# Arash-san/YinYang-Game-AlphaZero

Hardware: AMD Instinct MI355X
Metric: self-play positions/sec (+ MCTS node-expansions/sec) at 800 sims, 8x8 board (higher is better)
Workload: dtype f16x3; 1 GPU; 8x8 board, 800 sims/move, 4096 concurrent games per GPU, frozen random-init 128x10 net (seed 0), copied boards, reference_quirks=False, staggered start plies; tree_arithmetic=f32 PUCT + u64 bitboards, nn_dtype=f16x3, evaluation_reuse=False, parallelism=episode-sharded x1, lanes_per_gpu=2, hipgraph=True

## Files before the change

include/yy_engine.h:

```cpp
#ifndef YY_ENGINE_H
#define YY_ENGINE_H

#include <stdint.h>

#ifdef __cplusplus
extern "C" {
#endif

#define YY_OK 0
#define YY_E_INVALID (-1)
#define YY_E_UNSUPPORTED (-2)
#define YY_E_NOMEM (-3)
#define YY_E_HIP (-4)
#define YY_E_STATE (-5)
#define YY_E_ARENA (-6)

#define YY_FLAG_ROWCOL 1u
#define YY_FLAG_ALIASED 2u
#define YY_FLAG_REUSE_PASS_VALUE 4u

#define YY_FLAG_REUSE_TRANSPOSITIONS 8u
#define YY_FLAG_KEEP_EVALUATIONS 16u

#define YY_FLAG_EVAL_SYMMETRY 32u

#define YY_FLAG_FORCED_PLAYOUTS 64u

#define YY_FLAG_FPU_REDUCTION 128u

typedef void *yy_stream_t;

const char *yy_last_error(void);
int yy_version(void);


int yy_rules_valid_mask(const int8_t *boards, const int8_t *players, int G, int R, int C,
                        uint32_t flags, uint8_t *out_mask, yy_stream_t stream);

int yy_rules_step(int8_t *boards, int8_t *players, const int32_t *actions, int G, int R, int C,
                  uint32_t flags, uint8_t *placed, yy_stream_t stream);

int yy_rules_game_ended(const int8_t *boards, const int8_t *players, int G, int R, int C,
                        uint32_t flags, double *out, int32_t *counts, yy_stream_t stream);

int yy_encode_planes(const int8_t *boards, int G, int R, int C, float *out, yy_stream_t stream);

int yy_encode_planes_sym(const int8_t *boards, int G, int R, int C, uint64_t seed, float *out, yy_stream_t stream);
int yy_eval_symmetry(const int8_t *boards, int G, int R, int C, uint64_t seed, int8_t *out, yy_stream_t stream);

int yy_rules_mask_terminal_bb(const uint64_t *black, const uint64_t *white, int G, int R, int C,
                              uint32_t flags, uint64_t *mask_p1, uint64_t *mask_m1,
                              int8_t *result, yy_stream_t stream);

int yy_pack_boards(const int8_t *boards, int G, int R, int C, uint64_t *black, uint64_t *white,
                   yy_stream_t stream);
int yy_unpack_boards(const uint64_t *black, const uint64_t *white, int G, int R, int C,
                     int8_t *boards, yy_stream_t stream);


typedef struct yy_mcts_config {
    int32_t G;
    int32_t R, C;
    int32_t max_sims;
    float cpuct;
    uint32_t flags;
    int64_t edges_per_game;
    int64_t nodes_per_game;
    int32_t leaves_per_step;
    uint64_t symmetry_seed;
    double forced_playouts;
    float fpu_reduction;
    float fpu_reduction_root;
} yy_mcts_config;


typedef struct yy_mcts yy_mcts;

int yy_mcts_create(const yy_mcts_config *cfg, yy_mcts **out);
int yy_mcts_destroy(yy_mcts *ctx);
int yy_mcts_memory_bytes(const yy_mcts *ctx, uint64_t *out);
int yy_mcts_set_num_sims(yy_mcts *ctx, int32_t num_sims);
int yy_mcts_set_sim_budgets(yy_mcts *ctx, const int32_t *budgets_dev);

int yy_mcts_advance(yy_mcts *ctx, const int32_t *actions, int32_t *kept_visits, yy_stream_t stream);

int yy_mcts_begin(yy_mcts *ctx, const int8_t *boards, const int8_t *root_players,
                  const uint8_t *active, float *planes_out, yy_stream_t stream);

int yy_mcts_expand_root(yy_mcts *ctx, const float *policy, const double *noise, double eps,
                        yy_stream_t stream);

int yy_mcts_select(yy_mcts *ctx, float *planes_out, uint8_t *needs_eval, yy_stream_t stream);

int yy_mcts_expand_backup(yy_mcts *ctx, const float *policy, const float *value,
                          yy_stream_t stream);

int yy_mcts_step(yy_mcts *ctx, const float *policy, const float *value, float *planes_out,
                 uint8_t *needs_eval, yy_stream_t stream);

int yy_mcts_root_counts(yy_mcts *ctx, int32_t *counts, float *child_w, float *child_p,
                        yy_stream_t stream);

int yy_mcts_root_policy(yy_mcts *ctx, int temperature_is_zero, double *pi, yy_stream_t stream);

int yy_mcts_root_stats(yy_mcts *ctx, int32_t *visits, double *value_sum, yy_stream_t stream);

int yy_mcts_get_boards(yy_mcts *ctx, int8_t *boards, yy_stream_t stream);

int yy_mcts_status(yy_mcts *ctx, int32_t *n_overflow, uint64_t *counters);
int yy_mcts_reset_counters(yy_mcts *ctx, yy_stream_t stream);
int yy_mcts_forced_descents(yy_mcts *ctx, uint64_t *out);
int yy_book_insert(const uint64_t *keys, int n, int R, int C, uint32_t *meta, uint64_t *table_keys, int64_t cap,
                   int32_t *slot_of, yy_stream_t stream);
int yy_mcts_set_book(yy_mcts *ctx, const uint32_t *meta, const uint64_t *keys, const float *value, const float *policy,
                     int64_t cap, int max_stones);
int yy_mcts_cache_clear(yy_mcts *ctx, yy_stream_t stream);
int yy_mcts_set_shared_evaluations(yy_mcts *ctx, uint32_t *meta, uint64_t *keys, float *value, float *policy, int64_t slots,
                                   uint32_t *stamp);
int yy_mcts_shared_evaluations_clear(yy_mcts *ctx, yy_stream_t stream);
int yy_mcts_shared_counters(yy_mcts *ctx, uint64_t *out);
int yy_mcts_set_shared_evaluations_replacing(yy_mcts *ctx, uint64_t *claim, uint32_t *last_hit, uint64_t *keys, float *value,
                                             float *policy, int64_t slots, uint32_t *stamp, uint64_t *sweep_state);
int yy_mcts_shared_evaluations_sweep(yy_mcts *ctx, int64_t high_water_slots, yy_stream_t stream);
int yy_mcts_shared_counters_ex(yy_mcts *ctx, uint64_t *out);

int yy_nn_bias_act_bf16(void *x, const float *bias, const void *residual, int64_t rows, int C,
                        int relu, yy_stream_t stream);

int yy_nn_tower_bf16(const float *planes, const void *weights, const float *bias, void *out, int G,
                     int R, int C, int channels, int n_layers, yy_stream_t stream);

int yy_nn_tower_heads_bf16(const float *planes, const void *weights, const float *bias,
                           void *out_heads, int G, int R, int C, int channels, int n_layers,
                           yy_stream_t stream);

int yy_nn_tower_f32(const float *planes, const void *weights, const float *bias, float *out, int G,
                    int R, int C, int channels, int n_layers, yy_stream_t stream);

int yy_nn_head_finish_bf16(const void *h, int G, int A, int H, const float *w2, const float *b2,
                           float *policy, float *value, yy_stream_t stream);

int yy_nn_tower_f16x3_regs(const float *planes, const void *weights, const void *head_w, const float *bias,
                           float *out, float *out_heads, const int32_t *rows, const int32_t *n_rows, int G,
                           int R, int C, int channels, int n_layers, int weight_exp, int head_exp,
                           int act_exp, yy_stream_t stream);

int yy_nn_tower_g(const float *planes, const void *weights, const void *head_w, const float *bias, const float *head_bias,
                  float *out, float *out_heads, const int32_t *rows, const int32_t *n_rows, int G, int R, int C,
                  int channels, int n_layers, int weight_exp, int head_exp, int act_exp, int nb, int boards, int gate_lo,
                  int gate_hi, int layout, yy_stream_t stream);
int yy_nn_tower_g_forms(int channels, int *nb_out);
int yy_nn_tower_g_relu_check(uint32_t start, uint32_t count, uint32_t *counts, yy_stream_t stream);

int yy_nn_fc_heads_f16x3(const float *feats, const void *wpk, const float *bias, const int32_t *jobs, int n_jobs,
                         float *logits, float *hidden, const int32_t *n_rows, int G, int K, int A, int H,
                         int weight_exp, int act_exp, yy_stream_t stream);

int yy_nn_head_finish_f32(const float *logits, const float *hidden, int G, int A, int H, const float *w2,
                          const float *b2, const int32_t *rows, const int32_t *n_rows, float *policy,
                          float *value, yy_stream_t stream);

int yy_compact_rows(const uint8_t *flags, int G, int32_t *rows, int32_t *n, yy_stream_t stream);

int yy_selfplay_root_noise(uint64_t seed, const int64_t *game_id, const int32_t *ply, const uint8_t *draw,
                           const uint8_t *mask, int G, int A, double alpha, double *noise, yy_stream_t stream);

int yy_selfplay_sample_actions(uint64_t seed, const int64_t *game_id, const int32_t *ply,
                               const uint8_t *searching, const double *pi, const uint8_t *mask, int G, int A,
                               int temperature_threshold, int32_t *action, yy_stream_t stream);

int yy_selfplay_draw_budgets(uint64_t seed, const int64_t *game_id, const int32_t *ply, const uint8_t *searching, int G,
                             double p_full, int full_sims, int fast_sims, int32_t *budgets, uint8_t *is_full,
                             yy_stream_t stream);

typedef struct yy_selfplay_config {
    uint64_t seed;
    double dirichlet_alpha;
    double dirichlet_epsilon;
    double full_search_probability;
    int32_t temperature_threshold;
    int32_t num_simulations;
    int32_t fast_simulations;
    int32_t reserved;
    int64_t example_capacity;
} yy_selfplay_config;

typedef struct yy_selfplay_run yy_selfplay_run;

int yy_selfplay_run_create(yy_mcts *ctx, const yy_selfplay_config *cfg, yy_selfplay_run **out);
int yy_selfplay_run_destroy(yy_selfplay_run *run);
int yy_selfplay_run_arm(yy_mcts *ctx, yy_selfplay_run *run, int64_t num_games, int64_t first_game_index, int64_t stride,
                        float *planes, uint8_t *needs_eval, yy_stream_t stream);
int yy_mcts_step_selfplay(yy_mcts *ctx, yy_selfplay_run *run, const float *policy, const float *value, float *planes,
                          uint8_t *needs_eval, yy_stream_t stream);
int yy_selfplay_run_counters(yy_selfplay_run *run, uint64_t *out, yy_stream_t stream);
int yy_selfplay_run_examples(yy_selfplay_run *run, int64_t first, int64_t count, int8_t *states, float *policies,
                             float *values, int64_t *game_id, int64_t *ply, yy_stream_t stream);

#ifdef __cplusplus
}
#endif
#endif
```

yinyang-game-alphazero_amd/_lib.py:

```python
import ctypes as C
import os
import subprocess

_HERE = os.path.dirname(os.path.abspath(__file__))
CSRC = os.path.join(_HERE, "csrc")
SO = os.path.join(CSRC, "libyy_hip.so")
HEADER = os.path.normpath(os.path.join(_HERE, "..", "include", "yy_engine.h"))

YY_OK = 0
YY_E_ARENA = -6
FLAG_ROWCOL = 1
FLAG_ALIASED = 2
FLAG_REUSE_PASS_VALUE = 4
FLAG_REUSE_TRANSPOSITIONS = 8
FLAG_KEEP_EVALUATIONS = 16
FLAG_EVAL_SYMMETRY = 32
FLAG_FORCED_PLAYOUTS = 64
FLAG_FPU_REDUCTION = 128

HIPCC_FLAGS = ["--offload-arch=gfx950", "-O3", "-std=c++17", "-fPIC", "-shared",
               "-ffp-contract=off", "-fno-fast-math", "-Wall", "-Wno-unused-function"]


class YYError(RuntimeError):
    def __init__(self, code, msg):
        super().__init__(f"libyy_hip: status {code}: {msg}")
        self.code = code


class MctsConfig(C.Structure):
    _fields_ = [("G", C.c_int32), ("R", C.c_int32), ("C", C.c_int32), ("max_sims", C.c_int32),
                ("cpuct", C.c_float), ("flags", C.c_uint32), ("edges_per_game", C.c_int64),
                ("nodes_per_game", C.c_int64), ("leaves_per_step", C.c_int32), ("symmetry_seed", C.c_uint64),
                ("forced_playouts", C.c_double), ("fpu_reduction", C.c_float), ("fpu_reduction_root", C.c_float)]


class SelfPlayConfig(C.Structure):
    _fields_ = [("seed", C.c_uint64), ("dirichlet_alpha", C.c_double), ("dirichlet_epsilon", C.c_double),
                ("full_search_probability", C.c_double), ("temperature_threshold", C.c_int32),
                ("num_simulations", C.c_int32), ("fast_simulations", C.c_int32), ("reserved", C.c_int32),
                ("example_capacity", C.c_int64)]


def build(force=False, verbose=False):
    srcs = [os.path.join(CSRC, f) for f in ("yy_engine.hip", "yy_nn_epilogue.hip", "yy_tower.hip", "yy_tower_f32.hip",
                                            "yy_tower_h3r.hip", "yy_tower_g.hip", "yy_fc_heads.hip", "yy_selfplay.hip",
                                            "yy_selfplay_move.hip", "yy_shared_table.hip", "yy_bitboard.h", "yy_common.h", "yy_tree.h",
                                            "yy_draws.h")] + [HEADER]
    if not force and os.path.exists(SO) and all(os.path.getmtime(SO) >= os.path.getmtime(s) for s in srcs):
        return SO
    hipcc = os.environ.get("HIPCC", "/opt/rocm/bin/hipcc")
    tmp = f"{SO}.{os.getpid()}.tmp"
    cmd = [hipcc] + HIPCC_FLAGS + ["-o", tmp] + [s for s in srcs if s.endswith(".hip")]
    if verbose:
        print(" ".join(cmd).replace(tmp, SO))
    try:
        subprocess.check_call(cmd)
        os.replace(tmp, SO)
    finally:
        if os.path.exists(tmp):
            os.remove(tmp)
    return SO


_LIB = None
_vp = C.c_void_p
_SIGS = {
    "yy_rules_valid_mask": [_vp, _vp, C.c_int, C.c_int, C.c_int, C.c_uint32, _vp, _vp],
    "yy_rules_step": [_vp, _vp, _vp, C.c_int, C.c_int, C.c_int, C.c_uint32, _vp, _vp],
    "yy_rules_game_ended": [_vp, _vp, C.c_int, C.c_int, C.c_int, C.c_uint32, _vp, _vp, _vp],
    "yy_encode_planes": [_vp, C.c_int, C.c_int, C.c_int, _vp, _vp],
    "yy_encode_planes_sym": [_vp, C.c_int, C.c_int, C.c_int, C.c_uint64, _vp, _vp],
    "yy_eval_symmetry": [_vp, C.c_int, C.c_int, C.c_int, C.c_uint64, _vp, _vp],
    "yy_rules_mask_terminal_bb": [_vp, _vp, C.c_int, C.c_int, C.c_int, C.c_uint32, _vp, _vp, _vp, _vp],
    "yy_pack_boards": [_vp, C.c_int, C.c_int, C.c_int, _vp, _vp, _vp],
    "yy_unpack_boards": [_vp, _vp, C.c_int, C.c_int, C.c_int, _vp, _vp],
    "yy_mcts_create": [C.POINTER(MctsConfig), C.POINTER(_vp)],
    "yy_mcts_destroy": [_vp],
    "yy_mcts_memory_bytes": [_vp, C.POINTER(C.c_uint64)],
    "yy_mcts_set_num_sims": [_vp, C.c_int32],
    "yy_mcts_set_sim_budgets": [_vp, _vp],
    "yy_mcts_advance": [_vp, _vp, _vp, _vp],
    "yy_mcts_begin": [_vp, _vp, _vp, _vp, _vp, _vp],
    "yy_mcts_expand_root": [_vp, _vp, _vp, C.c_double, _vp],
    "yy_mcts_select": [_vp, _vp, _vp, _vp],
    "yy_mcts_expand_backup": [_vp, _vp, _vp, _vp],
    "yy_mcts_step": [_vp, _vp, _vp, _vp, _vp, _vp],
    "yy_mcts_root_counts": [_vp, _vp, _vp, _vp, _vp],
    "yy_mcts_root_policy": [_vp, C.c_int, _vp, _vp],
    "yy_mcts_root_stats": [_vp, _vp, _vp, _vp],
    "yy_mcts_get_boards": [_vp, _vp, _vp],
    "yy_mcts_status": [_vp, C.POINTER(C.c_int32), C.POINTER(C.c_uint64)],
    "yy_mcts_reset_counters": [_vp, _vp],
    "yy_mcts_forced_descents": [_vp, C.POINTER(C.c_uint64)],
    "yy_mcts_cache_clear": [_vp, _vp],
    "yy_book_insert": [_vp, C.c_int, C.c_int, C.c_int, _vp, _vp, C.c_int64, _vp, _vp],
    "yy_mcts_set_book": [_vp, _vp, _vp, _vp, _vp, C.c_int64, C.c_int],
    "yy_mcts_set_shared_evaluations": [_vp, _vp, _vp, _vp, _vp, C.c_int64, _vp],
    "yy_mcts_shared_evaluations_clear": [_vp, _vp],
    "yy_mcts_shared_counters": [_vp, C.POINTER(C.c_uint64)],
    "yy_mcts_set_shared_evaluations_replacing": [_vp, _vp, _vp, _vp, _vp, _vp, C.c_int64, _vp, _vp],
    "yy_mcts_shared_evaluations_sweep": [_vp, C.c_int64, _vp],
    "yy_mcts_shared_counters_ex": [_vp, C.POINTER(C.c_uint64)],
    "yy_nn_bias_act_bf16": [_vp, _vp, _vp, C.c_int64, C.c_int, C.c_int, _vp],
    "yy_nn_tower_bf16": [_vp, _vp, _vp, _vp, C.c_int, C.c_int, C.c_int, C.c_int, C.c_int, _vp],
    "yy_nn_tower_heads_bf16": [_vp, _vp, _vp, _vp, C.c_int, C.c_int, C.c_int, C.c_int, C.c_int, _vp],
    "yy_nn_head_finish_bf16": [_vp, C.c_int, C.c_int, C.c_int, _vp, _vp, _vp, _vp, _vp],
    "yy_nn_tower_f32": [_vp, _vp, _vp, _vp, C.c_int, C.c_int, C.c_int, C.c_int, C.c_int, _vp],
    "yy_nn_head_finish_f32": [_vp, _vp, C.c_int, C.c_int, C.c_int, _vp, _vp, _vp, _vp, _vp, _vp, _vp],
    "yy_compact_rows": [_vp, C.c_int, _vp, _vp, _vp],
    "yy_nn_tower_f16x3_regs": [_vp, _vp, _vp, _vp, _vp, _vp, _vp, _vp, C.c_int, C.c_int, C.c_int, C.c_int, C.c_int, C.c_int, C.c_int,
                               C.c_int, _vp],
    "yy_nn_tower_g_forms": [C.c_int, C.POINTER(C.c_int)],
    "yy_nn_tower_g_relu_check": [C.c_uint32, C.c_uint32, _vp, _vp],
    "yy_nn_tower_g": [_vp, _vp, _vp, _vp, _vp, _vp, _vp, _vp, _vp, C.c_int, C.c_int, C.c_int, C.c_int, C.c_int, C.c_int, C.c_int,
                      C.c_int, C.c_int, C.c_int, C.c_int, C.c_int, C.c_int, _vp],
    "yy_nn_fc_heads_f16x3": [_vp, _vp, _vp, _vp, C.c_int, _vp, _vp, _vp, C.c_int, C.c_int, C.c_int, C.c_int, C.c_int, C.c_int, _vp],
    "yy_selfplay_root_noise": [C.c_uint64, _vp, _vp, _vp, _vp, C.c_int, C.c_int, C.c_double, _vp, _vp],
    "yy_selfplay_sample_actions": [C.c_uint64, _vp, _vp, _vp, _vp, _vp, C.c_int, C.c_int, C.c_int, _vp, _vp],
    "yy_selfplay_draw_budgets": [C.c_uint64, _vp, _vp, _vp, C.c_int, C.c_double, C.c_int, C.c_int, _vp, _vp, _vp],
    "yy_selfplay_run_create": [_vp, C.POINTER(SelfPlayConfig), C.POINTER(_vp)],
    "yy_selfplay_run_destroy": [_vp],
    "yy_selfplay_run_arm": [_vp, _vp, C.c_int64, C.c_int64, C.c_int64, _vp, _vp, _vp],
    "yy_mcts_step_selfplay": [_vp, _vp, _vp, _vp, _vp, _vp, _vp],
    "yy_selfplay_run_counters": [_vp, _vp, _vp],
    "yy_selfplay_run_examples": [_vp, C.c_int64, C.c_int64, _vp, _vp, _vp, _vp, _vp, _vp],
    "yy_version": [],
}


def exported_symbols():
    return sorted(list(_SIGS) + ["yy_last_error"])


def lib():
    global _LIB
    if _LIB is None:
        if not os.path.exists(SO):
            raise YYError(-100, f"{SO} is missing: run __graft_entry__.build() (hipcc --offload-arch=gfx950); "
                                "there is no CPU fallback for the product path")
        L = C.CDLL(SO)
        for name, args in _SIGS.items():
            fn = getattr(L, name)
            fn.argtypes = args
            fn.restype = C.c_int
        L.yy_last_error.restype = C.c_char_p
        L.yy_last_error.argtypes = []
        _LIB = L
    return _LIB


def check(status):
    if status != YY_OK:
        raise YYError(status, lib().yy_last_error().decode())
    return status
```

yinyang-game-alphazero_amd/csrc/yy_fc_heads.hip:

```cpp
#include <hip/hip_runtime.h>
#include <math.h>
#include <stdint.h>

#include "../../include/yy_engine.h"

typedef __attribute__((ext_vector_type(8))) _Float16 f16x8;
typedef __attribute__((ext_vector_type(2))) _Float16 f16x2;
typedef __attribute__((ext_vector_type(4))) float f32x4;
typedef __attribute__((ext_vector_type(2))) float f32x2;
typedef __attribute__((ext_vector_type(4))) unsigned int u32x4;
typedef __attribute__((ext_vector_type(2))) unsigned int u32x2;

#include "yy_common.h"

namespace fch {

constexpr int KC = 128, RS = 288;

__device__ __forceinline__ void split_pair(const f32x2 a, uint32_t &hi, uint32_t &lo) {
    const f16x2 h = __builtin_convertvector(a, f16x2);
    const f32x2 r = a - __builtin_convertvector(h, f32x2);
    const f16x2 l = __builtin_convertvector(r, f16x2);
    hi = __builtin_bit_cast(uint32_t, h);
    lo = __builtin_bit_cast(uint32_t, l);
}

struct Job {
    int head, out0, nout, wchunk;
};

template <int ROWS>
__global__ void __launch_bounds__(256, 2)
k_fc_heads(const float *__restrict__ feats, const unsigned char *__restrict__ wpk, const float *__restrict__ bias,
           const Job *__restrict__ jobs, int n_jobs, float *__restrict__ logits, float *__restrict__ hidden,
           const int *__restrict__ n_rows, int G, int K, int A, int H, float in_scale, float out_scale) {
    constexpr int PART_BYTES = ROWS * RS, STAGE_BYTES = 2 * PART_BYTES, NBR = ROWS / 16, NI = ROWS / 8;
    __shared__ __attribute__((aligned(256))) unsigned char lds[2 * STAGE_BYTES];
    const int n_live = n_rows ? min(*n_rows, G) : G;
    const int tile = blockIdx.x / n_jobs, jb = blockIdx.x - tile * n_jobs;
    const int r0 = tile * ROWS;
    if (r0 >= n_live) return;
    const Job job = jobs[jb];
    const int lane = threadIdx.x & 63, wave = __builtin_amdgcn_readfirstlane(threadIdx.x >> 6);
    const int n16 = lane & 15, kg = lane >> 4;
    const int n_chunks = (K + KC - 1) / KC;
    const bool active = wave * 16 < job.nout;

    const int sq = threadIdx.x & 31, sr = threadIdx.x >> 5;
    auto stage_load = [&](f32x4 (&fr)[NI], int c) {
        const int k = c * KC + sq * 4;
        const int kc = k < K ? k : 0;
        const float km = k < K ? 1.0f : 0.0f;
#pragma unroll
        for (int i = 0; i < NI; i++) {
            const int row = min(r0 + sr + 8 * i, n_live - 1);
            fr[i] = *(const f32x4 *)(feats + ((size_t)row * 2 + job.head) * K + kc) * km;
        }
    };
    auto stage_store = [&](const f32x4 (&fr)[NI], int s) {
        unsigned char *base = lds + s * STAGE_BYTES + sq * 8;
#pragma unroll
        for (int i = 0; i < NI; i++) {
            const f32x4 v = fr[i] * in_scale;
            uint32_t h01, l01, h23, l23;
            split_pair((f32x2){v[0], v[1]}, h01, l01);
            split_pair((f32x2){v[2], v[3]}, h23, l23);
            *(u32x2 *)(base + (sr + 8 * i) * RS) = (u32x2){h01, h23};
            *(u32x2 *)(base + PART_BYTES + (sr + 8 * i) * RS) = (u32x2){l01, l23};
        }
    };
    const unsigned char *wbase = wpk + ((size_t)job.wchunk * 4 + wave) * 2048 + lane * 16;
    f32x4 acc1[NBR], acc2[NBR];
#pragma unroll
    for (int nb = 0; nb < NBR; nb++) acc1[nb] = acc2[nb] = (f32x4){0.f, 0.f, 0.f, 0.f};

    auto load_wc = [&](f16x8 (&w)[KC / 32][2], int c) {
#pragma unroll
        for (int ks = 0; ks < KC / 32; ks++) {
            const unsigned char *p = wbase + (size_t)(c * (KC / 32) + ks) * 8192;
            w[ks][0] = __builtin_bit_cast(f16x8, *(const u32x4 *)p);
            w[ks][1] = __builtin_bit_cast(f16x8, *(const u32x4 *)(p + 1024));
        }
    };
    auto compute = [&](const f16x8 (&w)[KC / 32][2], int stage) {
        if (!active) return;
        const unsigned char *xs = lds + stage * STAGE_BYTES + n16 * RS + kg * 16;
        constexpr int NG = (KC / 32) * NBR, P = 4;
        f16x8 xh[P], xl[P];
        auto rd = [&](int g, int slot) {
            const int ks = g / NBR, nb = g % NBR;
            xh[slot] = __builtin_bit_cast(f16x8, *(const u32x4 *)(xs + nb * 16 * RS + ks * 64));
            xl[slot] = __builtin_bit_cast(f16x8, *(const u32x4 *)(xs + PART_BYTES + nb * 16 * RS + ks * 64));
        };
#pragma unroll
        for (int g = 0; g < P; g++) rd(g, g);
        __builtin_amdgcn_sched_group_barrier(0x100, 2 * P, 0);
#pragma unroll
        for (int g = 0; g < NG; g++) {
            const int ks = g / NBR, nb = g % NBR, slot = g % P;
            const f32x4 a = __builtin_amdgcn_mfma_f32_16x16x32_f16(w[ks][1], xh[slot], acc2[nb], 0, 0, 0);
            acc1[nb] = __builtin_amdgcn_mfma_f32_16x16x32_f16(w[ks][0], xh[slot], acc1[nb], 0, 0, 0);
            acc2[nb] = __builtin_amdgcn_mfma_f32_16x16x32_f16(w[ks][0], xl[slot], a, 0, 0, 0);
            if (g + P < NG) rd(g + P, slot);
            __builtin_amdgcn_sched_group_barrier(0x008, 3, 0);
            __builtin_amdgcn_sched_group_barrier(0x100, 2, 0);
        }
    };
    const int last = n_chunks - 1;
    f32x4 f0[NI], f1[NI];
    f16x8 w0[KC / 32][2], w1[KC / 32][2];
    stage_load(f1, 0);
    load_wc(w0, 0);
    stage_load(f0, min(1, last));
    load_wc(w1, min(1, last));
    stage_store(f1, 0);
    stage_load(f1, min(2, last));
    __syncthreads();
    for (int c = 0; c < n_chunks; c += 2) {
        compute(w0, 0);
        if (c + 1 < n_chunks) stage_store(f0, 1);
        stage_load(f0, min(c + 3, last));
        load_wc(w0, min(c + 2, last));
        __syncthreads();
        if (c + 1 >= n_chunks) break;
        compute(w1, 1);
        if (c + 2 < n_chunks) stage_store(f1, 0);
        stage_load(f1, min(c + 4, last));
        load_wc(w1, min(c + 3, last));
        __syncthreads();
    }
    if (!active) return;
    float *out = job.head == 0 ? logits : hidden;
    const int W = job.head == 0 ? A : H, boff = job.head == 0 ? 0 : A;
    const int o0 = job.out0 + wave * 16 + kg * 4;
    float b[4];
#pragma unroll
    for (int i = 0; i < 4; i++) b[i] = (o0 + i < job.out0 + job.nout) ? bias[boff + o0 + i] : 0.0f;
#pragma unroll
    for (int nb = 0; nb < NBR; nb++) {
        const int row = r0 + nb * 16 + n16;
        if (row < n_live) {
#pragma unroll
            for (int i = 0; i < 4; i++)
                if (o0 + i < job.out0 + job.nout) out[(size_t)row * W + o0 + i] = __builtin_fmaf(acc1[nb][i] + acc2[nb][i], out_scale, b[i]);
        }
    }
}

}

extern "C" int yy_nn_fc_heads_f16x3(const float *feats, const void *wpk, const float *bias, const int32_t *jobs, int n_jobs,
                                    float *logits, float *hidden, const int32_t *n_rows, int G, int K, int A, int H,
                                    int weight_exp, int act_exp, yy_stream_t s) {
    if (G == 0) return YY_OK;
    if (!feats || !wpk || !bias || !jobs || !logits || !hidden || G < 0 || n_jobs < 1 || K < 32 || (K & 31) || A < 1 || H < 1)
        return yy_tower_set_err(YY_E_INVALID, "yy_nn_fc_heads_f16x3: bad argument");
    const float in_scale = ldexpf(1.0f, act_exp), out_scale = ldexpf(1.0f, -(weight_exp + act_exp));
    if (G <= 2048)
        fch::k_fc_heads<32><<<dim3(((G + 31) / 32) * n_jobs), dim3(256), 0, (hipStream_t)s>>>(
            feats, (const unsigned char *)wpk, bias, (const fch::Job *)jobs, n_jobs, logits, hidden, n_rows, G, K, A, H, in_scale, out_scale);
    else
        fch::k_fc_heads<64><<<dim3(((G + 63) / 64) * n_jobs), dim3(256), 0, (hipStream_t)s>>>(
            feats, (const unsigned char *)wpk, bias, (const fch::Job *)jobs, n_jobs, logits, hidden, n_rows, G, K, A, H, in_scale, out_scale);
    if (hipGetLastError() != hipSuccess) return yy_tower_set_err(YY_E_HIP, "yy_nn_fc_heads_f16x3: launch failed");
    return YY_OK;
}
```

yinyang-game-alphazero_amd/engine.py:

```python
import ctypes as ct

import numpy as np
import torch

from . import _lib
from .options import SHARED_EVALUATIONS_DEFAULT_SLOTS, SHARED_EVALUATIONS_HIGH_WATER, forced_k, fpu_r, shared_slots
from ._lib import FLAG_ALIASED, FLAG_EVAL_SYMMETRY, FLAG_FORCED_PLAYOUTS, FLAG_FPU_REDUCTION, FLAG_REUSE_PASS_VALUE, FLAG_KEEP_EVALUATIONS, FLAG_REUSE_TRANSPOSITIONS, FLAG_ROWCOL, MctsConfig, check, lib


def _stream():
    return ct.c_void_p(torch.cuda.current_stream().cuda_stream)


def _p(t):
    return None if t is None else ct.c_void_p(t.data_ptr())


def _need(t, dtype, shape=None, name="tensor"):
    if not isinstance(t, torch.Tensor) or not t.is_cuda:
        raise _lib.YYError(-1, f"{name}: expected a ROCm device tensor (the hot path has no CPU fallback)")
    if t.dtype != dtype or not t.is_contiguous():
        raise _lib.YYError(-1, f"{name}: expected contiguous {dtype}, got {t.dtype} contiguous={t.is_contiguous()}")
    if shape is not None and tuple(t.shape) != tuple(shape):
        raise _lib.YYError(-1, f"{name}: expected shape {tuple(shape)}, got {tuple(t.shape)}")
# ... 62 lines not shown

def evaluation_symmetry(boards, seed):
    G, R, Cc = boards.shape
    _need(boards, torch.int8, name="boards")
    out = torch.empty(G, dtype=torch.int8, device=boards.device)
    with torch.cuda.device(boards.device):
        check(lib().yy_eval_symmetry(_p(boards), G, R, Cc, _u64(seed), _p(out), _stream()))
    return out


def pack_boards(boards):
    G, R, Cc = boards.shape
    _need(boards, torch.int8, name="boards")
    nw = (R * Cc + 63) // 64
    black = torch.empty((nw, G), dtype=torch.int64, device=boards.device)
    white = torch.empty((nw, G), dtype=torch.int64, device=boards.device)
    with torch.cuda.device(boards.device):
        check(lib().yy_pack_boards(_p(boards), G, R, Cc, _p(black), _p(white), _stream()))
    return black, white


def unpack_boards(black, white, R, Cc):
    nw, G = black.shape
    _need(black, torch.int64, name="black")
    _need(white, torch.int64, (nw, G), "white")
    boards = torch.empty((G, R, Cc), dtype=torch.int8, device=black.device)
    with torch.cuda.device(black.device):
        check(lib().yy_unpack_boards(_p(black), _p(white), G, R, Cc, _p(boards), _stream()))
    return boards


def mask_terminal_bb(black, white, R, Cc, rowcol=False, out=None):
    nw, G = black.shape
    _need(black, torch.int64, name="black")
    _need(white, torch.int64, (nw, G), "white")
    if out is None:
        out = (torch.empty_like(black), torch.empty_like(black),
               torch.empty(G, dtype=torch.int8, device=black.device))
    m1, m2, res = out
    with torch.cuda.device(black.device):
        check(lib().yy_rules_mask_terminal_bb(_p(black), _p(white), G, R, Cc, _flags(rowcol), _p(m1), _p(m2), _p(res), _stream()))
    return m1, m2, res


def bias_act_(x, bias, residual=None, relu=True):
    if x.dim() != 4 or not x.is_contiguous(memory_format=torch.channels_last) or x.dtype != torch.bfloat16 or not x.is_cuda:
        raise _lib.YYError(-1, "bias_act_: expected a channels-last bf16 device tensor [N,C,H,W]")
    N, Cc, H, W = x.shape
    if bias.dtype != torch.float32 or bias.numel() != Cc or not bias.is_cuda:
        raise _lib.YYError(-1, "bias_act_: bias must be float32 [C] on the device")
    if residual is not None and (residual.shape != x.shape or residual.dtype != x.dtype
                                 or not residual.is_contiguous(memory_format=torch.channels_last)):
        raise _lib.YYError(-1, "bias_act_: residual must match x (channels-last bf16)")
    with torch.cuda.device(x.device):
        check(lib().yy_nn_bias_act_bf16(_p(x), _p(bias), _p(residual), N * H * W, Cc, int(bool(relu)), _stream()))
    return x


def tower_forward(planes, weights, bias, n_layers):
    G, _, R, Cc = planes.shape
    _need(planes, torch.float32, (G, 5, R, Cc), "planes")
    n_chunks = 9 + 18 * (n_layers - 1)
    _need(weights, torch.int16, (n_chunks, 8192), "tower weights")
    _need(bias, torch.float32, (n_layers, 128), "tower bias")
    out = torch.empty((G, R, Cc, 128), dtype=torch.bfloat16, device=planes.device)
    with torch.cuda.device(planes.device):
        check(lib().yy_nn_tower_bf16(_p(planes), _p(weights), _p(bias), _p(out), G, R, Cc, 128, n_layers, _stream()))
    return out.permute(0, 3, 1, 2)


def tower_forward_f32(planes, weights, bias, n_layers):
    G = planes.shape[0]
    _need(planes, torch.float32, (G, 5, 8, 8), "planes")
    _need(weights, torch.float32, (9 + 36 * (n_layers - 1), 4096), "f32 tower weights")
    _need(bias, torch.float32, (n_layers, 128), "tower bias")
    out = torch.empty((G, 8, 8, 128), dtype=torch.float32, device=planes.device)
    with torch.cuda.device(planes.device):
        check(lib().yy_nn_tower_f32(_p(planes), _p(weights), _p(bias), _p(out), G, 8, 8, 128, n_layers, _stream()))
    return out.permute(0, 3, 1, 2)


def tower_heads_forward_h3r(planes, weights, head_w, bias, n_layers, exps, rows=None, n_rows=None, out=None):
    G, _, R, Cc = planes.shape
    _need(planes, torch.float32, (G, 5, R, Cc), "planes")
    _need(weights, torch.int16, (9 + 36 * (n_layers - 1), 8192), "wave-major split-f16 tower weights")
    _need(head_w, torch.int16, (2, 8192), "wave-major split-f16 head weights")
    _need(bias, torch.float32, (n_layers + 1, 128), "tower+heads bias")
    if rows is not None:
        _need(rows, torch.int32, (G,), "rows")
        _need(n_rows, torch.int32, (1,), "n_rows")
    if out is None:
        out = torch.empty((G, 2, 32 * R * Cc), dtype=torch.float32, device=planes.device)
    _need(out, torch.float32, (G, 2, 32 * R * Cc), "out")
    with torch.cuda.device(planes.device):
        check(lib().yy_nn_tower_f16x3_regs(_p(planes), _p(weights), _p(head_w), _p(bias), None, _p(out), _p(rows), _p(n_rows), G, R, Cc,
                                           128, n_layers, int(exps[0]), int(exps[1]), int(exps[2]), _stream()))
    return out


def tower_forward_h3r(planes, weights, bias, n_layers, exps):
    G, _, R, Cc = planes.shape
    _need(planes, torch.float32, (G, 5, R, Cc), "planes")
    _need(weights, torch.int16, (9 + 36 * (n_layers - 1), 8192), "wave-major split-f16 tower weights")
    _need(bias, torch.float32, (n_layers, 128), "tower bias")
    out = torch.empty((G, R, Cc, 128), dtype=torch.float32, device=planes.device)
    with torch.cuda.device(planes.device):
        check(lib().yy_nn_tower_f16x3_regs(_p(planes), _p(weights), None, _p(bias), _p(out), None, None, None, G, R, Cc, 128, n_layers,
                                           int(exps[0]), 0, int(exps[2]), _stream()))
    return out.permute(0, 3, 1, 2)


def tower_g_available(channels):
    buf = (ct.c_int * 8)()
    n = lib().yy_nn_tower_g_forms(int(channels), buf)
    return [int(buf[i]) for i in range(n)]


def tower_g(planes, weights, bias, n_layers, exps, nb, boards, head_w=None, head_bias=None, rows=None, n_rows=None, out=None,
            gate=(-1, 0x7FFFFFFF), column_layout=False, wave_grid=True):
    G, _, R, Cc = planes.shape
    _need(planes, torch.float32, (G, 5, R, Cc), "planes")
    ch = bias.shape[1]
    nw = ch // 32
    _need(weights, torch.int16, (9 + 9 * nw * (n_layers - 1), ch * 64), "split-f16 tower weights (pack_tower_g)")
    _need(bias, torch.float32, (n_layers, ch), "tower bias")
    if rows is not None:
        _need(rows, torch.int32, (G,), "rows")
        _need(n_rows, torch.int32, (1,), "n_rows")
    heads = head_w is not None
    if heads:
        _need(head_w, torch.int16, (4 * nw * 2 * 512,), "split-f16 head weights (pack_heads_g)")
        _need(head_bias, torch.float32, (64,), "head bias")
        if out is None:
            out = torch.empty((G, 2, 32 * R * Cc), dtype=torch.float32, device=planes.device)
        _need(out, torch.float32, (G, 2, 32 * R * Cc), "out")
    else:
        out = torch.empty((G, R, Cc, ch), dtype=torch.float32, device=planes.device)
    with torch.cuda.device(planes.device):
        check(lib().yy_nn_tower_g(_p(planes), _p(weights), _p(head_w), _p(bias), _p(head_bias), None if heads else _p(out),
                                  _p(out) if heads else None, _p(rows), _p(n_rows), G, R, Cc, ch, n_layers, int(exps[0]), int(exps[1]),
                                  int(exps[2]), int(nb), int(boards), int(gate[0]), int(gate[1]),
                                  1 if column_layout else 0 if wave_grid else 2,
                                  _stream()))
    return out if heads else out.permute(0, 3, 1, 2)


def tower_g_relu_check(start, count, counts):
    _need(counts, torch.int32, (2,), "counts")
    with torch.cuda.device(counts.device):
        check(lib().yy_nn_tower_g_relu_check(int(start) & 0xFFFFFFFF, int(count), _p(counts), _stream()))
    return counts


def fc_heads(feats, wpk, bias, jobs, A, H, exps, n_rows=None, logits=None, hidden=None):
    G, two, K = feats.shape
    _need(feats, torch.float32, (G, 2, K), "feats")
    _need(jobs, torch.int32, (jobs.shape[0], 4), "jobs")
    ksteps = ((K + 127) // 128) * 4
    _need(wpk, torch.int16, (jobs.shape[0] * ksteps * 4096,), "fc head weights (pack_fc_heads)")
    _need(bias, torch.float32, (A + H,), "fc head bias")
    if n_rows is not None:
        _need(n_rows, torch.int32, (1,), "n_rows")
    if logits is None:
        logits = torch.empty((G, A), dtype=torch.float32, device=feats.device)
        hidden = torch.empty((G, H), dtype=torch.float32, device=feats.device)
    _need(logits, torch.float32, (G, A), "logits")
    _need(hidden, torch.float32, (G, H), "hidden")
    with torch.cuda.device(feats.device):
        check(lib().yy_nn_fc_heads_f16x3(_p(feats), _p(wpk), _p(bias), _p(jobs), jobs.shape[0], _p(logits), _p(hidden), _p(n_rows), G, K,
                                         A, H, int(exps[0]), int(exps[1]), _stream()))
    return logits, hidden


def head_finish_f32(logits, hidden, w2, b2, rows=None, n_rows=None, policy=None, value=None):
    G, A = logits.shape
    _need(logits, torch.float32, name="logits")
    _need(hidden, torch.float32, (G, hidden.shape[1]), "hidden")
    _need(w2, torch.float32, (hidden.shape[1],), "w2")
    _need(b2, torch.float32, (1,), "b2")
    if rows is not None:
        _need(rows, torch.int32, (G,), "rows")
        _need(n_rows, torch.int32, (1,), "n_rows")
    if policy is None:
        policy = torch.zeros((G, A), dtype=torch.float32, device=logits.device)
        value = torch.zeros(G, dtype=torch.float32, device=logits.device)
    _need(policy, torch.float32, (G, A), "policy")
    _need(value, torch.float32, (G,), "value")
    with torch.cuda.device(logits.device):
        check(lib().yy_nn_head_finish_f32(_p(logits), _p(hidden), G, A, hidden.shape[1], _p(w2), _p(b2), _p(rows), _p(n_rows),
                                          _p(policy), _p(value), _stream()))
    return policy, value


def compact_rows(flags, rows=None, n=None):
    G = flags.shape[0]
    _need(flags, torch.uint8, (G,), "flags")
    if rows is None:
        rows = torch.zeros(G, dtype=torch.int32, device=flags.device)
        n = torch.zeros(1, dtype=torch.int32, device=flags.device)
    _need(rows, torch.int32, (G,), "rows")
    _need(n, torch.int32, (1,), "n")
    with torch.cuda.device(flags.device):
        check(lib().yy_compact_rows(_p(flags), G, _p(rows), _p(n), _stream()))
    return rows, n


def tower_heads_forward(planes, weights, bias, n_layers):
    G, _, R, Cc = planes.shape
    _need(planes, torch.float32, (G, 5, R, Cc), "planes")
    n_chunks = 9 + 18 * (n_layers - 1) + 1
    _need(weights, torch.int16, (n_chunks, 8192), "tower+heads weights")
    _need(bias, torch.float32, (n_layers + 1, 128), "tower+heads bias")
    out = torch.empty((G, 2, 32 * R * Cc), dtype=torch.bfloat16, device=planes.device)
    with torch.cuda.device(planes.device):
        check(lib().yy_nn_tower_heads_bf16(_p(planes), _p(weights), _p(bias), _p(out), G, R, Cc, 128, n_layers, _stream()))
    return out


def head_finish(h, A, w2, b2):
    G, W = h.shape
    _need(h, torch.bfloat16, name="h")
    _need(w2, torch.float32, (W - A,), "w2")
    _need(b2, torch.float32, (1,), "b2")
    policy = torch.empty((G, A), dtype=torch.float32, device=h.device)
    value = torch.empty(G, dtype=torch.float32, device=h.device)
    with torch.cuda.device(h.device):
        check(lib().yy_nn_head_finish_bf16(_p(h), G, A, W - A, _p(w2), _p(b2), _p(policy), _p(value), _stream()))
    return policy, value


def root_noise(seed, game_id, ply, draw, mask, alpha):
    G, A = mask.shape
    _need(game_id, torch.int64, (G,), "game_id")
    _need(ply, torch.int32, (G,), "ply")
    _need(draw, torch.uint8, (G,), "draw")
    _need(mask, torch.uint8, (G, A), "mask")
    out = torch.empty((G, A), dtype=torch.float64, device=mask.device)
    with torch.cuda.device(mask.device):
        check(lib().yy_selfplay_root_noise(ct.c_uint64(int(seed) & (2 ** 64 - 1)), _p(game_id), _p(ply), _p(draw), _p(mask), G, A,
                                           float(alpha), _p(out), _stream()))
    return out


def sample_actions(seed, game_id, ply, searching, pi, mask, temperature_threshold):
    G, A = mask.shape
    _need(game_id, torch.int64, (G,), "game_id")
    _need(ply, torch.int32, (G,), "ply")
    _need(searching, torch.uint8, (G,), "searching")
    _need(pi, torch.float64, (G, A), "pi")
    _need(mask, torch.uint8, (G, A), "mask")
    out = torch.empty(G, dtype=torch.int32, device=mask.device)
    with torch.cuda.device(mask.device):
        check(lib().yy_selfplay_sample_actions(ct.c_uint64(int(seed) & (2 ** 64 - 1)), _p(game_id), _p(ply), _p(searching), _p(pi),
                                               _p(mask), G, A, int(temperature_threshold), _p(out), _stream()))
    return out


def draw_budgets(seed, game_id, ply, searching, p_full, full_sims, fast_sims):
    G = game_id.shape[0]
    _need(game_id, torch.int64, (G,), "game_id")
    _need(ply, torch.int32, (G,), "ply")
    _need(searching, torch.uint8, (G,), "searching")
    budgets = torch.empty(G, dtype=torch.int32, device=game_id.device)
    is_full = torch.empty(G, dtype=torch.uint8, device=game_id.device)
    with torch.cuda.device(game_id.device):
        check(lib().yy_selfplay_draw_budgets(ct.c_uint64(int(seed) & (2 ** 64 - 1)), _p(game_id), _p(ply), _p(searching), G,
                                             float(p_full), int(full_sims), int(fast_sims), _p(budgets), _p(is_full), _stream()))
    return budgets, is_full


class SelfPlayRun:

    COUNTERS = ("started", "finished", "failed", "positions", "recorded", "rows", "overflow", "target")

    def __init__(self, ctx, seed, num_simulations, example_capacity, dirichlet_alpha=0.3, dirichlet_epsilon=0.25,
                 temperature_threshold=10, fast_simulations=None, full_search_probability=1.0):
        self.ctx, self.capacity = ctx, int(example_capacity)
        cfg = _lib.SelfPlayConfig(int(seed) & (2 ** 64 - 1), float(dirichlet_alpha), float(dirichlet_epsilon),
                                  float(full_search_probability), int(temperature_threshold), int(num_simulations),
                                  int(fast_simulations or 0), 0, self.capacity)
        h = ct.c_void_p()
        with torch.cuda.device(ctx.device):
            check(lib().yy_selfplay_run_create(ctx._h, ct.byref(cfg), ct.byref(h)))
        self._h = h
        self.host, self._flip = torch.zeros((2, len(self.COUNTERS)), dtype=torch.int64).pin_memory(), 0

    def close(self):
        if getattr(self, "_h", None) is not None and self._h.value:
            torch.cuda.synchronize(self.ctx.device)
            lib().yy_selfplay_run_destroy(self._h)
            self._h = None

    def __del__(self):
        try:
            self.close()
        except Exception:
            pass

    def arm(self, num_games, first_game_index=0, stride=1):
        ctx = self.ctx
        with torch.cuda.device(ctx.device):
            check(lib().yy_selfplay_run_arm(ctx._h, self._h, int(num_games), int(first_game_index), int(stride), _p(ctx.planes),
                                            _p(ctx.needs_eval), _stream()))

    def step(self, policy, value):
        ctx = self.ctx
        _need(policy, torch.float32, (ctx.rows, ctx.A), "policy")
        _need(value, torch.float32, (ctx.rows,), "value")
        with torch.cuda.device(ctx.device):
            check(lib().yy_mcts_step_selfplay(ctx._h, self._h, _p(policy), _p(value), _p(ctx.planes), _p(ctx.needs_eval), _stream()))

    def poll_counters(self):
        self._flip ^= 1
        host = self.host[self._flip]
        with torch.cuda.device(self.ctx.device):
            check(lib().yy_selfplay_run_counters(self._h, ct.c_void_p(host.data_ptr()), _stream()))
        event = torch.cuda.Event()
        event.record()
        return event, host

    def counters(self, host):
        return dict(zip(self.COUNTERS, (int(x) for x in host.tolist())))

# ... 422 lines not shown
```

Baseline: 1875 positions/s.

## Add one-pass FC heads kernel processing two output slices per workgroup

Measured after the change: 1875 positions/s, median of 2. Within noise of the previous version (+0.0%).

```diff
diff --git a/include/yy_engine.h b/include/yy_engine.h
--- a/include/yy_engine.h
+++ b/include/yy_engine.h
@@ -155,6 +155,9 @@
 int yy_nn_fc_heads_f16x3(const float *feats, const void *wpk, const float *bias, const int32_t *jobs, int n_jobs,
                          float *logits, float *hidden, const int32_t *n_rows, int G, int K, int A, int H,
                          int weight_exp, int act_exp, yy_stream_t stream);
+int yy_nn_fc_heads_f16x3_form(const float *feats, const void *wpk, const float *bias, const int32_t *jobs, int n_jobs,
+                              float *logits, float *hidden, const int32_t *n_rows, int G, int K, int A, int H,
+                              int weight_exp, int act_exp, int form, yy_stream_t stream);
 
 int yy_nn_head_finish_f32(const float *logits, const float *hidden, int G, int A, int H, const float *w2,
                           const float *b2, const int32_t *rows, const int32_t *n_rows, float *policy,
diff --git a/yinyang-game-alphazero_amd/_lib.py b/yinyang-game-alphazero_amd/_lib.py
--- a/yinyang-game-alphazero_amd/_lib.py
+++ b/yinyang-game-alphazero_amd/_lib.py
@@ -116,6 +116,8 @@
     "yy_nn_tower_g": [_vp, _vp, _vp, _vp, _vp, _vp, _vp, _vp, _vp, C.c_int, C.c_int, C.c_int, C.c_int, C.c_int, C.c_int, C.c_int,
                       C.c_int, C.c_int, C.c_int, C.c_int, C.c_int, C.c_int, _vp],
     "yy_nn_fc_heads_f16x3": [_vp, _vp, _vp, _vp, C.c_int, _vp, _vp, _vp, C.c_int, C.c_int, C.c_int, C.c_int, C.c_int, C.c_int, _vp],
+    "yy_nn_fc_heads_f16x3_form": [_vp, _vp, _vp, _vp, C.c_int, _vp, _vp, _vp, C.c_int, C.c_int, C.c_int, C.c_int, C.c_int, C.c_int,
+                                  C.c_int, _vp],
     "yy_selfplay_root_noise": [C.c_uint64, _vp, _vp, _vp, _vp, C.c_int, C.c_int, C.c_double, _vp, _vp],
     "yy_selfplay_sample_actions": [C.c_uint64, _vp, _vp, _vp, _vp, _vp, C.c_int, C.c_int, C.c_int, _vp, _vp],
     "yy_selfplay_draw_budgets": [C.c_uint64, _vp, _vp, _vp, C.c_int, C.c_double, C.c_int, C.c_int, _vp, _vp, _vp],
diff --git a/yinyang-game-alphazero_amd/csrc/yy_fc_heads.hip b/yinyang-game-alphazero_amd/csrc/yy_fc_heads.hip
--- a/yinyang-game-alphazero_amd/csrc/yy_fc_heads.hip
+++ b/yinyang-game-alphazero_amd/csrc/yy_fc_heads.hip
@@ -147,21 +147,202 @@
     }
 }
 
-}
-
-extern "C" int yy_nn_fc_heads_f16x3(const float *feats, const void *wpk, const float *bias, const int32_t *jobs, int n_jobs,
-                                    float *logits, float *hidden, const int32_t *n_rows, int G, int K, int A, int H,
-                                    int weight_exp, int act_exp, yy_stream_t s) {
+template <int ROWS, int NSL, int WGS>
+__device__ __forceinline__ void
+heads_once_body(unsigned char *lds, const Job (&js)[NSL], const bool active, const float *__restrict__ feats, const unsigned char *__restrict__ wpk,
+                const float *__restrict__ bias, float *__restrict__ logits, float *__restrict__ hidden, int n_live, int r0,
+                int K, int A, int H, float in_scale, float out_scale) {
+    constexpr int PART_BYTES = ROWS * RS, STAGE_BYTES = 2 * PART_BYTES, NBR = ROWS / 16, NI = ROWS / (8 * WGS), KS = KC / 32;
+    static_assert(NI >= 1 && NI * 8 * WGS == ROWS, "the workgroup's threads stage whole passes of 8 * WGS rows");
+    constexpr int WD = NSL <= 2 ? 2 : 1;
+    const int head = js[0].head;
+    const int lane = threadIdx.x & 63, wave = __builtin_amdgcn_readfirstlane(threadIdx.x >> 6) & 3;
+    const int n16 = lane & 15, kg = lane >> 4;
+    const int n_chunks = (K + KC - 1) / KC, last = n_chunks - 1;
+
+    const int sq = threadIdx.x & 31, sr = threadIdx.x >> 5;
+    auto stage_load = [&](f32x4 (&fr)[NI], int c) {
+        const int k = c * KC + sq * 4;
+        const int kc = k < K ? k : 0;
+        const float km = k < K ? 1.0f : 0.0f;
+#pragma unroll
+        for (int i = 0; i < NI; i++) {
+            const int row = min(r0 + sr + 8 * WGS * i, n_live - 1);
+            fr[i] = *(const f32x4 *)(feats + ((size_t)row * 2 + head) * K + kc) * km;
+        }
+    };
+    auto stage_store = [&](const f32x4 (&fr)[NI], int s) {
+        unsigned char *base = lds + s * STAGE_BYTES + sq * 8;
+#pragma unroll
+        for (int i = 0; i < NI; i++) {
+            const f32x4 v = fr[i] * in_scale;
+            uint32_t h01, l01, h23, l23;
+            split_pair((f32x2){v[0], v[1]}, h01, l01);
+            split_pair((f32x2){v[2], v[3]}, h23, l23);
+            *(u32x2 *)(base + (sr + 8 * WGS * i) * RS) = (u32x2){h01, h23};
+            *(u32x2 *)(base + PART_BYTES + (sr + 8 * WGS * i) * RS) = (u32x2){l01, l23};
+        }
+    };
+    const unsigned char *wbase[NSL];
+    f32x4 acc1[NSL][NBR], acc2[NSL][NBR];
+#pragma unroll
+    for (int s = 0; s < NSL; s++) {
+        wbase[s] = wpk + ((size_t)js[s].wchunk * 4 + wave) * 2048 + lane * 16;
+#pragma unroll
+        for (int nb = 0; nb < NBR; nb++) acc1[s][nb] = acc2[s][nb] = (f32x4){0.f, 0.f, 0.f, 0.f};
+    }
+    auto load_wk = [&](f16x8 (&w)[NSL][2], int c, int ks) {
+#pragma unroll
+        for (int s = 0; s < NSL; s++) {
+            const unsigned char *p = wbase[s] + (size_t)(c * KS + ks) * 8192;
+            w[s][0] = __builtin_bit_cast(f16x8, *(const u32x4 *)p);
+            w[s][1] = __builtin_bit_cast(f16x8, *(const u32x4 *)(p + 1024));
+        }
+    };
+    auto compute = [&](f16x8 (&w)[KS][NSL][2], int stage, int c_next) {
+        if (!active) return;
+        const unsigned char *xs = lds + stage * STAGE_BYTES + n16 * RS + kg * 16;
+        constexpr int NG = KS * NBR, P = 4;
+        f16x8 xh[P], xl[P];
+        auto rd = [&](int g, int slot) {
+            const int ks = g / NBR, nb = g % NBR;
+            xh[slot] = __builtin_bit_cast(f16x8, *(const u32x4 *)(xs + nb * 16 * RS + ks * 64));
+            xl[slot] = __builtin_bit_cast(f16x8, *(const u32x4 *)(xs + PART_BYTES + nb * 16 * RS + ks * 64));
+        };
+#pragma unroll
+        for (int g = 0; g < P && g < NG; g++) rd(g, g);
+        __builtin_amdgcn_sched_group_barrier(0x100, 2 * (P < NG ? P : NG), 0);
+#pragma unroll
+        for (int g = 0; g < NG; g++) {
+            const int ks = g / NBR, nb = g % NBR, slot = g % P;
+#pragma unroll
+            for (int s = 0; s < NSL; s++) {
+                const f32x4 a = __builtin_amdgcn_mfma_f32_16x16x32_f16(w[ks][s][1], xh[slot], acc2[s][nb], 0, 0, 0);
+                acc1[s][nb] = __builtin_amdgcn_mfma_f32_16x16x32_f16(w[ks][s][0], xh[slot], acc1[s][nb], 0, 0, 0);
+                acc2[s][nb] = __builtin_amdgcn_mfma_f32_16x16x32_f16(w[ks][s][0], xl[slot], a, 0, 0, 0);
+            }
+            if (g + P < NG) rd(g + P, slot);
+            __builtin_amdgcn_sched_group_barrier(0x008, 3 * NSL, 0);
+            __builtin_amdgcn_sched_group_barrier(0x100, 2, 0);
+            if (nb == NBR - 1) load_wk(w[ks], c_next, ks);
+        }
+    };
+    f32x4 f0[NI], f1[NI];
+    f16x8 w[WD][KS][NSL][2];
+    stage_load(f1, 0);
+#pragma unroll
+    for (int d = 0; d < WD; d++)
+#pragma unroll
+        for (int ks = 0; ks < KS; ks++)
+            if (active) load_wk(w[d][ks], min(d, last), ks);
+    stage_load(f0, min(1, last));
+    stage_store(f1, 0);
+    stage_load(f1, min(2, last));
+    __syncthreads();
+    for (int c = 0; c < n_chunks; c += 2) {
+        compute(w[0], 0, min(c + WD, last));
+        if (c + 1 < n_chunks) stage_store(f0, 1);
+        stage_load(f0, min(c + 3, last));
+        __syncthreads();
+        if (c + 1 >= n_chunks) break;
+        compute(w[WD - 1], 1, min(c + 1 + WD, last));
+        if (c + 2 < n_chunks) stage_store(f1, 0);
+        stage_load(f1, min(c + 4, last));
+        __syncthreads();
+    }
+    if (!active) return;
+    float *out = head == 0 ? logits : hidden;
+    const int W = head == 0 ? A : H, boff = head == 0 ? 0 : A;
+#pragma unroll
+    for (int s = 0; s < NSL; s++) {
+        const int o0 = js[s].out0 + wave * 16 + kg * 4, oend = js[s].out0 + js[s].nout;
+        float b[4];
+#pragma unroll
+        for (int i = 0; i < 4; i++) b[i] = (o0 + i < oend) ? bias[boff + o0 + i] : 0.0f;
+#pragma unroll
+        for (int nb = 0; nb < NBR; nb++) {
+            const int row = r0 + nb * 16 + n16;
+            if (row < n_live) {
+#pragma unroll
+                for (int i = 0; i < 4; i++)
+                    if (o0 + i < oend) out[(size_t)row * W + o0 + i] = __builtin_fmaf(acc1[s][nb][i] + acc2[s][nb][i], out_scale, b[i]);
+            }
+        }
+    }
+}
+
+template <int ROWS, int NS, int OCC>
+__global__ void __launch_bounds__(256 * NS, OCC)
+k_fc_heads_once(const float *__restrict__ feats, const unsigned char *__restrict__ wpk, const float *__restrict__ bias,
+                const Job *__restrict__ jobs, int n_jobs, float *__restrict__ logits, float *__restrict__ hidden,
+                const int *__restrict__ n_rows, int G, int K, int A, int H, float in_scale, float out_scale) {
+    __shared__ __attribute__((aligned(256))) unsigned char lds[4 * ROWS * RS];
+    const int n_live = n_rows ? min(*n_rows, G) : G;
+    const int ng0 = ((A + 63) / 64 + NS - 1) / NS, ng = ng0 + ((H + 63) / 64 + NS - 1) / NS;
+    const int tile = blockIdx.x / ng, gi = blockIdx.x - tile * ng;
+    const int r0 = tile * ROWS;
+    if (r0 >= n_live) return;
+    const int head = gi >= ng0 ? 1 : 0, first = (gi - head * ng0) * NS;
+    Job js[NS];
+    int seen = 0;
+#pragma unroll
+    for (int s = 0; s < NS; s++) js[s] = Job{head, 0, 0, 0};
+    for (int j = 0; j < n_jobs; j++) {
+        const Job t = jobs[j];
+        if (t.head != head) continue;
+#pragma unroll
+        for (int s = 0; s < NS; s++)
+            if (seen == first + s) js[s] = t;
+        seen++;
+    }
+    const int wave = __builtin_amdgcn_readfirstlane(threadIdx.x >> 6), quad = wave >> 2;
+    Job mine[1] = {js[0]};
+#pragma unroll
+    for (int s = 1; s < NS; s++)
+        if (quad == s) mine[0] = js[s];
+    heads_once_body<ROWS, 1, NS>(lds, mine, (wave & 3) * 16 < mine[0].nout, feats, wpk, bias, logits, hidden, n_live, r0, K, A, H,
+                                 in_scale, out_scale);
+}
+
+}
+
+extern "C" int yy_nn_fc_heads_f16x3_form(const float *feats, const void *wpk, const float *bias, const int32_t *jobs, int n_jobs,
+                                         float *logits, float *hidden, const int32_t *n_rows, int G, int K, int A, int H,
+                                         int weight_exp, int act_exp, int form, yy_stream_t s) {
     if (G == 0) return YY_OK;
     if (!feats || !wpk || !bias || !jobs || !logits || !hidden || G < 0 || n_jobs < 1 || K < 32 || (K & 31) || A < 1 || H < 1)
         return yy_tower_set_err(YY_E_INVALID, "yy_nn_fc_heads_f16x3: bad argument");
     const float in_scale = ldexpf(1.0f, act_exp), out_scale = ldexpf(1.0f, -(weight_exp + act_exp));
-    if (G <= 2048)
-        fch::k_fc_heads<32><<<dim3(((G + 31) / 32) * n_jobs), dim3(256), 0, (hipStream_t)s>>>(
-            feats, (const unsigned char *)wpk, bias, (const fch::Job *)jobs, n_jobs, logits, hidden, n_rows, G, K, A, H, in_scale, out_scale);
-    else
-        fch::k_fc_heads<64><<<dim3(((G + 63) / 64) * n_jobs), dim3(256), 0, (hipStream_t)s>>>(
-            feats, (const unsigned char *)wpk, bias, (const fch::Job *)jobs, n_jobs, logits, hidden, n_rows, G, K, A, H, in_scale, out_scale);
+    const hipStream_t st = (hipStream_t)s;
+    const unsigned char *w = (const unsigned char *)wpk;
+    const fch::Job *jb = (const fch::Job *)jobs;
+#define YY_FCH_ONCE(ROWS, NS, OCC)                                                                                                 \
+    fch::k_fc_heads_once<ROWS, NS, OCC><<<dim3(((G + ROWS - 1) / ROWS) * (((A + 63) / 64 + NS - 1) / NS + ((H + 63) / 64 + NS - 1) / NS)), \
+                                          dim3(256 * NS), 0, st>>>(feats, w, bias, jb, n_jobs, logits, hidden, n_rows, G, K, A, H, in_scale, out_scale)
+    if (form != 0 && form != 1) return yy_tower_set_err(YY_E_INVALID, "yy_nn_fc_heads_f16x3: unknown form");
+    if (form == 0 && n_jobs != (A + 63) / 64 + (H + 63) / 64)
+        return yy_tower_set_err(YY_E_INVALID, "yy_nn_fc_heads_f16x3: job table does not cut the heads into slices of 64");
+    if (form == 1 || (G > 512 && G <= 1600)) {
+        if (G <= 2048)
+            fch::k_fc_heads<32><<<dim3(((G + 31) / 32) * n_jobs), dim3(256), 0, st>>>(
+                feats, w, bias, jb, n_jobs, logits, hidden, n_rows, G, K, A, H, in_scale, out_scale);
+        else
+            fch::k_fc_heads<64><<<dim3(((G + 63) / 64) * n_jobs), dim3(256), 0, st>>>(
+                feats, w, bias, jb, n_jobs, logits, hidden, n_rows, G, K, A, H, in_scale, out_scale);
+    } else if (G <= 512) {
+        YY_FCH_ONCE(16, 2, 2);
+    } else if (G <= 2688) {
+        YY_FCH_ONCE(32, 2, 2);
+    } else {
+        YY_FCH_ONCE(64, 2, 1);
+    }
+#undef YY_FCH_ONCE
     if (hipGetLastError() != hipSuccess) return yy_tower_set_err(YY_E_HIP, "yy_nn_fc_heads_f16x3: launch failed");
     return YY_OK;
 }
+
+extern "C" int yy_nn_fc_heads_f16x3(const float *feats, const void *wpk, const float *bias, const int32_t *jobs, int n_jobs,
+                                    float *logits, float *hidden, const int32_t *n_rows, int G, int K, int A, int H,
+                                    int weight_exp, int act_exp, yy_stream_t s) {
+    return yy_nn_fc_heads_f16x3_form(feats, wpk, bias, jobs, n_jobs, logits, hidden, n_rows, G, K, A, H, weight_exp, act_exp, 0, s);
+}
diff --git a/yinyang-game-alphazero_amd/engine.py b/yinyang-game-alphazero_amd/engine.py
--- a/yinyang-game-alphazero_amd/engine.py
+++ b/yinyang-game-alphazero_amd/engine.py
@@ -238,7 +238,7 @@
     return counts
 
 
-def fc_heads(feats, wpk, bias, jobs, A, H, exps, n_rows=None, logits=None, hidden=None):
+def fc_heads(feats, wpk, bias, jobs, A, H, exps, n_rows=None, logits=None, hidden=None, form=0):
     G, two, K = feats.shape
     _need(feats, torch.float32, (G, 2, K), "feats")
     _need(jobs, torch.int32, (jobs.shape[0], 4), "jobs")
@@ -253,8 +253,8 @@
     _need(logits, torch.float32, (G, A), "logits")
     _need(hidden, torch.float32, (G, H), "hidden")
     with torch.cuda.device(feats.device):
-        check(lib().yy_nn_fc_heads_f16x3(_p(feats), _p(wpk), _p(bias), _p(jobs), jobs.shape[0], _p(logits), _p(hidden), _p(n_rows), G, K,
-                                         A, H, int(exps[0]), int(exps[1]), _stream()))
+        check(lib().yy_nn_fc_heads_f16x3_form(_p(feats), _p(wpk), _p(bias), _p(jobs), jobs.shape[0], _p(logits), _p(hidden), _p(n_rows),
+                                              G, K, A, H, int(exps[0]), int(exps[1]), int(form), _stream()))
     return logits, hidden
 
 
```
